# chrhansk/pygradflow

Hardware: AMD Instinct MI355X
Metric: Newton steps/sec on dense KKT n=4096 m=1024; iterate match <=1e-10 (higher is better)
Workload: dtype f64; 1 GPU; dense_qp_n4096_m1024; n=4096, m=1024, newton_type=Full, step_solver=Symmetric, instances_per_gpu=1, collective=none

## Files before the change

include/pgf_hip.h:

```cpp
#ifndef PGF_HIP_H
#define PGF_HIP_H

#include <stdint.h>

#ifdef __cplusplus
extern "C" {
#endif

#define PGF_OK 0
#define PGF_SINGULAR 1
#define PGF_INERTIA 2
#define PGF_INVALID 3
#define PGF_NOT_READY 4
#define PGF_HIP_ERROR 100

#define PGF_HOST 0
#define PGF_DEVICE 1

#define PGF_CREATE_SPARSE 1u

#define PGF_STEP_RECOMPUTE_MASK 1u
#define PGF_STEP_REFACTOR 2u
#define PGF_STEP_REFACTOR_ON_CHANGE 4u

// ... 121 lines not shown
                     double *flops_out);

int pgf_kkt_apply(pgf_handle h, const double *v, double *out);

int pgf_set_refinement(pgf_handle h, int mode, double tol, double fail_tol);
int pgf_refinement_stats(pgf_handle h, int *refined, int *lu_fallbacks, double *last_rel_residual);

int pgf_debug_fail_next_chain(pgf_handle h);
int pgf_debug_chain_enable(int on);
int pgf_debug_fail_next_helper(pgf_handle h);
int pgf_batch_debug_fail_next_helper(pgf_batch b);
int pgf_debug_chain_helpers(int on);
int pgf_debug_factor_kind(pgf_handle h);
int pgf_batch_debug_factor_kind(pgf_batch b);
int pgf_debug_step_stats(pgf_handle h, int *host_syncs, int *redone_steps);

#ifdef __cplusplus
}
#endif
#endif
```

pygradflow_amd/_lib.py:

```python

from __future__ import annotations

import ctypes as C
import os
import sys

import numpy as np

from .errors import LinearSolverError

_HERE = os.path.dirname(os.path.abspath(__file__))
LIB_PATH = os.path.join(_HERE, "libpgf_hip.so")

PGF_OK, PGF_SINGULAR, PGF_INERTIA, PGF_INVALID, PGF_NOT_READY, PGF_HIP_ERROR = 0, 1, 2, 3, 4, 100
PGF_HOST, PGF_DEVICE = 0, 1
STEP_RECOMPUTE_MASK, STEP_REFACTOR, STEP_REFACTOR_ON_CHANGE = 1, 2, 4
CREATE_SPARSE = 1

_dp = C.POINTER(C.c_double)
_u8p = C.POINTER(C.c_uint8)
_ip = C.POINTER(C.c_int)
_h = C.c_void_p

SIGNATURES = {
# ... 57 lines not shown
    "pgf_ls_destroy": (C.c_int, [_h]),
    "pgf_bench_update": (C.c_int, [C.c_int, C.c_int, C.c_int, C.c_int, C.c_int, _dp, _dp]),
    "pgf_profile_read_ex": (C.c_int, [_h, _dp, C.c_int]),
    "pgf_batch_ctl_init": (C.c_int, [_h, C.c_double, C.c_double, _dp, C.c_int]),
    "pgf_batch_ctl_iterate": (C.c_int, [_h, C.c_uint, C.c_double, C.c_int]),
    "pgf_batch_ctl_read": (C.c_int, [_h, _dp, C.POINTER(C.c_uint8), _dp, C.c_int]),
    "pgf_kkt_apply": (C.c_int, [_h, _dp, _dp]),
    "pgf_set_refinement": (C.c_int, [_h, C.c_int, C.c_double, C.c_double]),
    "pgf_refinement_stats": (C.c_int, [_h, _ip, _ip, _dp]),
    "pgf_debug_fail_next_chain": (C.c_int, [_h]),
    "pgf_debug_chain_enable": (C.c_int, [C.c_int]),
    "pgf_debug_fail_next_helper": (C.c_int, [_h]),
    "pgf_debug_chain_helpers": (C.c_int, [C.c_int]),
    "pgf_debug_factor_kind": (C.c_int, [_h]),
    "pgf_debug_step_stats": (C.c_int, [_h, _ip, _ip]),
    "pgf_batch_refinement_stats": (C.c_int, [_h, _ip]),
    "pgf_comm_unique_id": (C.c_int, [C.c_void_p]),
    "pgf_comm_create": (C.c_int, [C.c_int, C.c_int, C.c_void_p, C.c_int, C.POINTER(C.c_void_p)]),
    "pgf_comm_destroy": (C.c_int, [C.c_void_p]),
    "pgf_batch_allgather_norms": (C.c_int, [_h, C.c_void_p, C.c_void_p]),
    "pgf_batch_debug_fail_next_helper": (C.c_int, [_h]),
    "pgf_batch_debug_factor_kind": (C.c_int, [_h]),
}

_lib = None


def load():
    global _lib
    if _lib is not None:
# ... 65 lines not shown
```

pygradflow_amd/csrc/pgf_api.hip:

```cpp
#include <cmath>
#include <cstdio>
#include <cstring>
#include <new>
#include <utility>

#include "../../include/pgf_hip.h"
#include "pgf_internal.h"
#include "pgf_kernels.h"
#include "pgf_sparse.h"

#define PGF_GEMVT_PARTS 32

#define STAT_COPY 16
#define STAT_ALLOC 17

struct pgf_solver {
  int n = 0, m = 0, device = 0;
  hipStream_t stream = nullptr;
  std::string err = "";
  double dt = 0, lamb = 0, rho = 0, fact = 0, delta = 0;
  bool bounds_set = false, outer_set = false, derivs_set = false, mask_set = false;
  bool qp_mode = false, point_set = false, eval_fresh = false;
  int nI = 0, nA = 0, N = 0;
  double *H = nullptr, *J = nullptr;
// ... 36 lines not shown
  bool sp_guarded = false;
  double *h_bred = nullptr;
  bool sp_stat_pending = false;
  double *stat = nullptr, *h_stat = nullptr;
  unsigned *ticket = nullptr;
  int stat_bits = 0;
  bool counts_known = false, spec_pending = false;
  bool step_took_inject = false;
  int stat_host_syncs = 0, stat_redone = 0;
  uint8_t *h_mask_stage = nullptr;
  hipEvent_t mask_ev = nullptr;
  bool fused_eval_done = false;
  bool condensed = false;
  bool condensed_veto = false;
  double *cd_t = nullptr;
};

struct pgf_linsolver {
  int N = 0, device = 0;
  bool symmetric = true;
  hipStream_t stream = nullptr;
  DenseLdlt fac;
  DenseLu lu;
  double *rhs = nullptr, *sol = nullptr;
};

static const char *k_no_handle = "null handle";
static const char *k_chain_msg = "chained triangular solve failed its placement / timeout check "
                                 "and so did the per-block solve that replaced it";

// ... 115 lines not shown
  }
  h->fac.prof = &h->prof;
  *out = h;
  return PGF_OK;
}

int pgf_destroy(pgf_handle h) {
  if (!h) return PGF_OK;
  (void)hipSetDevice(h->device);
  if (h->stream) (void)hipStreamSynchronize(h->stream);
  ldlt_chain_timing_dump();
  void *ptrs[] = {h->csr_ptr, h->csr_idx, h->csr_val, h->Hown, h->Jown, h->lb,  h->ub,   h->slb,  h->sub,      h->xhat, h->yhat,
                  h->x,    h->y,    h->xn,  h->yn,   h->g,    h->c,        h->F,    h->b0full,
                  h->rhs,  h->sol,  h->dx,  h->dy,   h->q,    h->b,        h->w,    h->tmpn,
                  h->partial, h->red, h->stat, h->mask, h->mask_new, h->idxI, h->idxA, h->pos,
                  h->meas, h->rs_v, h->rs_lv, h->rs_u, h->rs_wy, h->rs_r, h->rs_d, h->cd_t};
  for (void *p : ptrs)
    if (p) (void)hipFree(p);
  if (h->h_stat) (void)hipHostFree(h->h_stat);
  if (h->h_mask_stage) (void)hipHostFree(h->h_mask_stage);
  if (h->mask_ev) (void)hipEventDestroy(h->mask_ev);
  if (h->h_bred) (void)hipHostFree(h->h_bred);
  lu_free(h->lu);
  if (h->h_meas) (void)hipHostFree(h->h_meas);
  {
    SparseDev &sp = h->sp;
    void *sps[] = {sp.pos, sp.Hptr, sp.Hrow, sp.Hcol, sp.Hslot, sp.Jptr, sp.Jcol, sp.Jslot, sp.JTptr,
                   sp.JTrow, sp.JTmap, sp.Hval, sp.Jval, sp.band, sp.brhs, sp.Hb0, sp.Jb0,
                   sp.bD, sp.bL, sp.bU, sp.bDinv, sp.bF, sp.bneg, sp.brhs0, sp.bres, sp.bsol,
                   sp.bred};
    for (void *q : sps)
// ... 14 lines not shown
  return PGF_OK;
}

static int up(pgf_handle h, void *dst, const void *src, size_t bytes) {
  if (!bytes) return PGF_OK;
  HIPCHK(h, hipMemcpyAsync(dst, src, bytes, hipMemcpyHostToDevice, h->stream));
  return PGF_OK;
}

static int down(pgf_handle h, void *dst, const void *src, size_t bytes) {
  if (!bytes) return PGF_OK;
  HIPCHK(h, hipMemcpyAsync(dst, src, bytes, hipMemcpyDeviceToHost, h->stream));
  return PGF_OK;
}

static void invalidate_factor(pgf_handle h) {
  h->fac.factored = false;
  h->condensed_veto = false;
  h->lu_active = false;
  h->factor_clean = false;
}

int pgf_set_bounds(pgf_handle h, const double *lb, const double *ub) {
  if (!h) return PGF_INVALID;
  if (h->n && (!lb || !ub)) return fail(h, PGF_INVALID, "null bounds");
  (void)hipSetDevice(h->device);
  int rc;
  if ((rc = up(h, h->lb, lb, h->n * sizeof(double)))) return rc;
  if ((rc = up(h, h->ub, ub, h->n * sizeof(double)))) return rc;
  HIPCHK(h, hipStreamSynchronize(h->stream));
// ... 45 lines not shown
  HIPCHK(h, hipStreamSynchronize(h->stream));
  *cur = *own;
  *curld = cols;
  *owned = true;
  return PGF_OK;
}

int pgf_set_derivs_dense(pgf_handle h, const double *H, int64_t ldh, const double *J, int64_t ldj,
                         int loc) {
  if (!h) return PGF_INVALID;
  (void)hipSetDevice(h->device);
  int rc;
  if ((rc = set_matrix(h, H, ldh, h->n, h->n, loc, &h->Hown, &h->H, &h->ldh, &h->ownH))) return rc;
  if ((rc = set_matrix(h, J, ldj, h->m, h->n, loc, &h->Jown, &h->J, &h->ldj, &h->ownJ))) return rc;
  h->derivs_set = true;
  h->norms_valid = false;
  invalidate_factor(h);
  return PGF_OK;
}

static int csr_matrix_to_dense(pgf_handle h, int rows, int cols, const int *ptr, const int *idx,
                               const double *val, double **own, double **cur, int64_t *curld,
                               bool *owned) {
  if (rows == 0 || cols == 0) {
    *cur = nullptr;
    *curld = cols;
    return PGF_OK;
  }
  if (!ptr) return fail(h, PGF_INVALID, "null CSR row pointer");
  const int nnz = ptr[rows];
  if (ptr[0] != 0 || nnz < 0 || (nnz && (!idx || !val)))
// ... 35 lines not shown
}

int pgf_set_derivs_csr(pgf_handle h, const int *Hptr, const int *Hidx, const double *Hval,
                       const int *Jptr, const int *Jidx, const double *Jval) {
  if (!h) return PGF_INVALID;
  if (h->sparse) return fail(h, PGF_INVALID, "banded handles take pgf_sparse_set_pattern / _values");
  (void)hipSetDevice(h->device);
  int rc;
  if ((rc = csr_matrix_to_dense(h, h->n, h->n, Hptr, Hidx, Hval, &h->Hown, &h->H, &h->ldh,
                                &h->ownH)))
    return rc;
  if ((rc = csr_matrix_to_dense(h, h->m, h->n, Jptr, Jidx, Jval, &h->Jown, &h->J, &h->ldj,
                                &h->ownJ)))
    return rc;
  h->derivs_set = true;
  h->norms_valid = false;
  invalidate_factor(h);
  return PGF_OK;
}

static void tau_factors(pgf_handle h, double tau, int *use_tau, double *f_x, double *f_x0,
                        double *f_d) {
  *use_tau = std::isnan(tau) ? 0 : 1;
  const double lamb = 1.0 / h->dt;
  *f_x = *use_tau ? lamb * (1 - tau * lamb) : 0.0;
  *f_x0 = *use_tau ? tau * lamb * lamb : 0.0;
  *f_d = *use_tau ? tau * lamb : 0.0;
}

int pgf_active_set(pgf_handle h, const double *x, const double *g, double tau, uint8_t *mask_out) {
  if (!h) return PGF_INVALID;
// ... 139 lines not shown
    f.V = nullptr;
    f.vcap = 0;
    if ((e = hipMalloc((void **)&f.V, need * sizeof(double))) != hipSuccess) return e;
    f.vcap = need;
  }
  if (f.vdcap < (size_t)mp) {
    if (f.vd) (void)hipFree(f.vd);
    f.vd = nullptr;
    f.vdcap = 0;
    if ((e = hipMalloc((void **)&f.vd, (size_t)mp * sizeof(double))) != hipSuccess) return e;
    f.vdcap = mp;
  }
  return e;
}

static hipError_t kkt_solve_async(pgf_handle h, const double *rhs, double *sol) {
  if (!h->condensed) return ldlt_solve_async(h->fac, rhs, sol);
  DenseLdlt &f = h->fac;
  launch_cond_rhs(h->stream, h->nI, h->m, f.V, f.ldv, rhs, h->delta, h->cd_t);
  hipError_t e = ldlt_solve_async(f, h->cd_t, sol);
  if (e != hipSuccess) return e;
  launch_cond_y(h->stream, h->nI, h->m, f.V, f.ldv, sol, rhs + h->nI, h->delta, h->partial,
                (size_t)PGF_GEMVT_PARTS * (h->n ? h->n : 1), sol + h->nI);
  return hipGetLastError();
}
static hipError_t kkt_backsolve_async(pgf_handle h, double *sol) {
  DenseLdlt &f = h->fac;
  if (!h->condensed) return ldlt_backsolve_async(f, f.K + (int64_t)h->N * f.ldk, sol);
  hipError_t e = ldlt_backsolve_async(f, f.K + (int64_t)h->nI * f.ldk, sol);
  if (e != hipSuccess) return e;
// ... 22 lines not shown
  if (h->sparse) {
    sp_launch_assemble(h->stream, h->sp, h->n, h->m, h->mask, h->lamb, h->delta);
    if (sp_cyclic(h->sp)) {
      sp_cyclic_solve(h->stream, h->sp, h->n + h->m, h->fac.flags, false);
    } else {
      sp_launch_factor(h->stream, h->sp, h->n + h->m, h->fac.flags);
    }
    HIPCHK(h, hipMemcpyAsync(h->fac.h_flags, h->fac.flags, 4 * sizeof(int), hipMemcpyDeviceToHost,
                             h->stream));
    h->fac.factored = false;
    return PGF_OK;
  }
  h->lu_active = false;
  h->condensed = condensed_wanted(h);
  h->fac.vdepth = 0;
  if (h->condensed) {
    DenseLdlt &f = h->fac;
    HIPCHK(h, condensed_reserve(h));
    const int nI = h->nI, mp = (h->m + 31) / 32 * 32;
    f.ldv = condensed_ldv(h->m);
    f.vdepth = mp;
    f.vneg = h->m;
    f.flags_zeroed = nI > 0;
    launch_assemble_kkt(h->stream, f.K, f.ldk, h->H, h->ldh, h->J, h->ldj, h->idxI, nI, 0, h->lamb, h->delta,
                        f.flags, 4 + LDLT_UPD_COUNTERS, with_rhs ? h->rhs : nullptr,
                        f.K + (int64_t)nI * f.ldk, nI);
    launch_cond_panel(h->stream, f.V, f.ldv, mp, f.vd, h->J, h->ldj, h->idxI, nI, h->m, h->delta,
                      with_rhs ? h->rhs + nI : nullptr);
    HIPCHK(h, ldlt_factor_async(f, nI, nI + (with_rhs ? 1 : 0)));
    f.N = nI;
    return PGF_OK;
  }
  h->fac.flags_zeroed = h->N > 0;
  launch_assemble_kkt(h->stream, h->fac.K, h->fac.ldk, h->H, h->ldh, h->J, h->ldj, h->idxI, h->nI, h->m,
                      h->lamb, h->delta, h->fac.flags, 4 + LDLT_UPD_COUNTERS, with_rhs ? h->rhs : nullptr,
                      h->fac.K + (int64_t)h->N * h->fac.ldk, h->N);
  HIPCHK(h, ldlt_factor_async(h->fac, h->N, h->N + (with_rhs ? 1 : 0)));
  return PGF_OK;
}

#define PGF_RETRY_FACTOR (-2)
static int finish_factor_state(pgf_handle h, hipError_t *e) {
  const int st = ldlt_finish(h->fac, e);
  if (st == 1 && h->condensed && !h->condensed_veto) {
    h->condensed_veto = true;
    h->fac.factored = false;
    return 2;
  }
  return st;
}
static const char *k_helper_msg =
    "the dense factorisation failed its hand-over checks with and without helper workgroups";

static int sparse_status_sync(pgf_handle h) {
  if (!h->sparse || !h->sp_stat_pending) return PGF_OK;
  HIPCHK(h, hipStreamSynchronize(h->stream));
  h->sp_stat_pending = false;
  const int nr = h->sp.nred;
  double sum = 0.0;
  for (int i = 0; i < nr; ++i) sum += h->h_bred[2 * nr + i];
  h->h_scal[0] = sqrt(sum);
  for (int k = 0; k < 4; ++k) h->fac.h_flags[k] = (int)h->h_bred[3 * nr + k];
  return PGF_OK;
// ... 221 lines not shown
}

int pgf_factor(pgf_handle h, int *n_neg) {
  if (!h) return PGF_INVALID;
  int rc;
  if ((rc = check_ready(h))) return rc;
  (void)hipSetDevice(h->device);
  if ((rc = factor_sync(h))) return rc;
  if (n_neg) *n_neg = h->fac.n_neg;
  return PGF_OK;
}

static int newton_core_async(pgf_handle h, bool *did_factor) {
  hipStream_t s = h->stream;
  h->fused_eval_done = false;
  const bool rhs_fused = !h->sparse && h->nA == 0;
  if (rhs_fused)
    launch_residual_rhs(s, h->n, h->m, h->nI, h->lamb, h->dt, h->fact, h->xhat, h->yhat, h->x, h->y, h->g,
                        h->c, h->slb, h->sub, h->mask, h->idxI, h->F, h->b0full, h->rhs);
  else
    launch_residual(s, h->n, h->m, h->lamb, h->dt, h->xhat, h->yhat, h->x, h->y, h->g, h->c, h->slb,
                    h->sub, h->mask, h->F, h->b0full);
  if (h->sparse) {
    const int Nf = h->n + h->m;
    sp_launch_rhs(s, h->sp, h->n, h->m, h->mask, h->F, h->b0full, h->fact, h->sp.Hb0, h->sp.Jb0);
    *did_factor = false;
    if (sp_cyclic(h->sp)) {
      if (!h->fac.factored) sp_launch_assemble(s, h->sp, h->n, h->m, h->mask, h->lamb, h->delta);
      hipEvent_t e0 = nullptr, e1 = nullptr;
      if (h->prof.enabled) {
// ... 572 lines not shown
  if (!h->sparse) return down(h, h->h_stat, h->stat, STAT_COPY * sizeof(double));
  if (!h->sp_stat_pending) return down(h, h->h_scal, h->scal, sizeof(double));
  return PGF_OK;
}

static int settle_spec(pgf_handle h, bool *redone) {
  *redone = false;
  if (h->sparse || !h->step_pending || !h->spec_pending) return PGF_OK;
  h->spec_pending = false;
  if (!h->h_counts[3]) return PGF_OK;
  ++h->stat_redone;
  const int *w = reinterpret_cast<const int *>(h->h_stat + 14);
  ldlt_chain_discard(h->fac, (h->stat_bits & 2) ? w[3] : 0);
  h->stat_bits = 0;
  if (h->step_took_inject) h->fac.inject_helper_failure = 1;
  h->fac.factored = false;
  h->lu_active = false;
  std::swap(h->x, h->xn);
  std::swap(h->y, h->yn);
  h->eval_fresh = false;
  h->nI = h->h_counts[0];
  h->nA = h->h_counts[1];
  h->N = h->nI + h->m;
  int rc;
  if ((rc = enqueue_qp_step(h))) return rc;
  *redone = true;
  return PGF_OK;
}

int pgf_qp_step_async(pgf_handle h, unsigned policy, double tau) {
// ... 84 lines not shown
int pgf_debug_chain_enable(int on) {
  ldlt_chain_set_enabled(on != 0);
  return PGF_OK;
}

int pgf_debug_fail_next_helper(pgf_handle h) {
  if (!h) return PGF_INVALID;
  h->fac.inject_helper_failure = 1;
  return PGF_OK;
}

int pgf_debug_step_stats(pgf_handle h, int *host_syncs, int *redone_steps) {
  if (!h) return PGF_INVALID;
  if (host_syncs) *host_syncs = h->stat_host_syncs;
  if (redone_steps) *redone_steps = h->stat_redone;
  return PGF_OK;
}

int pgf_debug_factor_kind(pgf_handle h) {
  if (!h || h->sparse) return 0;
  if (h->lu_active) return 3;
  if (!h->fac.factored) return 0;
  return h->condensed ? 2 : 1;
}

int pgf_debug_chain_helpers(int on) {
  const int was = ldlt_chain_helpers_enabled() ? 1 : 0;
  if (on == 0 || on == 1) ldlt_chain_helpers_set(on == 1);
  return was;
}
// ... 520 lines not shown
static int batch_repair_instance(pgf_batch b, int i, double *diff_out) {
  pgf_handle h = b->hs[i];
  if (h->sparse || !h->refine_mode) return PGF_SINGULAR;
  const int nI = b->h_flags[3 * i + 2];
  h->nI = nI;
  h->nA = h->n - nI;
  h->N = nI + h->m;
  h->mask_set = true;
  h->condensed = b->cond_last;
  h->lu_active = false;
  h->last_solve = 2;
  DenseLdlt &f = h->fac;
  f.N = h->condensed ? nI : h->N;
  f.vdepth = h->condensed ? b->cond_mp : 0;
  f.ldv = condensed_ldv(h->m);
  f.vneg = h->m;
  f.factored = true;
  f.n_neg = b->h_flags[3 * i + 1] + (h->condensed ? h->m : 0);
  enqueue_residual(h);
  hipError_t e = hipStreamSynchronize(h->stream);
  if (e != hipSuccess) return hip_fail(h, e, "batched repair");
  int rc = refine_if_needed(h, false, false);
  if (rc) return rc;
  enqueue_step_update(h);
  launch_copy(h->stream, h->x, h->xn, h->n);
  launch_copy(h->stream, h->y, h->yn, h->m);
  if ((e = hipMemcpyAsync(h->h_scal, h->scal, sizeof(double), hipMemcpyDeviceToHost, h->stream)) != hipSuccess ||
      (e = hipStreamSynchronize(h->stream)) != hipSuccess)
    return hip_fail(h, e, "batched repair");
  if (ldlt_chain_check(f)) return fail(h, PGF_HIP_ERROR, k_chain_msg);
  *diff_out = h->h_scal[0];
// ... 499 lines not shown
```

pygradflow_amd/csrc/pgf_factor2.hip:

```cpp
#include <hip/hip_ext.h>

#include "pgf_internal.h"
#include "pgf_ldlt_dev.h"

#include <algorithm>
#include <atomic>
#include <cstdio>
#include <cstdlib>
#include <unordered_map>
#include <vector>

#define C_LD 66
#define C_WLD 18
#define CH_ROWS 256
#define CH_WAVES 16
#define CH_LT_OFF (CH_ROWS * C_LD * 8 + 2 * 64 * C_WLD * 8 + 3 * 64 * 8 + 16)
#define CH_SMEM (CH_LT_OFF + 2 * 16 * 16 * 8)

template <int TS>
__device__ __forceinline__ void tile_msub(double4_t &acc, double (*As)[C_LD], double (*Bs)[C_LD],
                                          const double *A, int64_t lda, int i0, int ilim,
                                          const double *B, int64_t ldb, int j0, int jlim, int kd) {
  constexpr int WPR = TS / 16, NT = 64 * WPR * WPR, NQ = TS * 32 / NT;
  const int tid = threadIdx.x, lane = tid & 63, wave = tid >> 6;
// ... 1935 lines not shown
    launch_t(c1, f.W + (size_t)(buf ^ 1) * f.wstride);
  }
  if (p) (void)hipEventRecord(p->factor_spans.back().second, s);
  if (f.inject_helper_failure) {
    f.inject_helper_failure = 0;
    hipLaunchKernelGGL(k_helper_inject, dim3(1), dim3(1), 0, s, f.flags);
  }
  if (f.defer_status) {
    f.status_words |= 1;
  } else {
    e = hipMemcpyAsync(f.h_flags, f.flags, 4 * sizeof(int), hipMemcpyDeviceToHost, s);
    if (e != hipSuccess) return e;
  }
  return hipGetLastError();
}
```

pygradflow_amd/csrc/pgf_internal.h:

```cpp
#pragma once

#include <hip/hip_runtime.h>
#include <stdint.h>

#include <string>
#include <vector>

#define PGF_NB 64

struct PgfProfile {
  bool enabled = false;
  int mode = 1;
  std::vector<std::pair<hipEvent_t, hipEvent_t>> fused_spans, trsmud_spans;
  std::vector<double> fused_flops, fused_bytes;
  double acc_fused_ms = 0, acc_fused_flops = 0, acc_fused_bytes = 0, acc_trsmud_ms = 0;
  int64_t acc_fused_launches = 0;
  std::vector<hipEvent_t> pool;
  std::vector<std::pair<hipEvent_t, hipEvent_t>> update_spans;
  std::vector<double> update_flops;
  std::vector<double> update_bytes;
  std::vector<std::pair<hipEvent_t, hipEvent_t>> factor_spans;
  std::vector<std::pair<hipEvent_t, hipEvent_t>> chain_spans, trsm_spans, udiag_spans;
  double acc_update_ms = 0, acc_update_flops = 0, acc_update_bytes = 0, acc_factor_ms = 0;
  double acc_chain_ms = 0, acc_trsm_ms = 0, acc_udiag_ms = 0;
// ... 30 lines not shown
  double *vd = nullptr;
  int vdepth = 0;
  int vneg = 0;
  size_t vcap = 0, vdcap = 0;
  int inject_chain_failure = 0;
  int inject_helper_failure = 0;
  bool flags_zeroed = false;
  bool defer_status = false;
  int status_words = 0;
};

hipError_t ldlt_alloc(DenseLdlt &f, int Nmax, hipStream_t stream);
void ldlt_free(DenseLdlt &f);
void ldlt_chain_discard(DenseLdlt &f, int word);
hipError_t ldlt_factor_async(DenseLdlt &f, int N, int nrows);
int ldlt_finish(DenseLdlt &f, hipError_t *err);
hipError_t ldlt_solve_async(DenseLdlt &f, const double *rhs, double *sol);
hipError_t ldlt_backsolve_async(DenseLdlt &f, const double *w, double *sol);
int ldlt_chain_check(DenseLdlt &f);
void ldlt_chain_set_enabled(bool on);
void ldlt_chain_helpers_off();
void ldlt_inject_helper_failure(hipStream_t s, int *flags);
bool ldlt_chain_helpers_enabled();
void ldlt_chain_helpers_set(bool on);
void ldlt_chain_timing_dump();
hipEvent_t prof_event(PgfProfile *p);

struct DenseLu {
  int N = 0;
  int64_t ld = 0;
// ... 110 lines not shown
```

pygradflow_amd/csrc/pgf_kernels.h:

```cpp
#pragma once

#include <hip/hip_runtime.h>
#include <stdint.h>

void launch_scale_bounds(hipStream_t s, int n, double lamb, const double *lb, const double *ub,
                         double *slb, double *sub);
void launch_active_set(hipStream_t s, int n, int use_tau, double lamb, double f_x, double f_x0,
                       double f_d, const double *xhat, const double *x, const double *g,
                       const double *slb, const double *sub, uint8_t *mask);
void launch_compact(hipStream_t s, int n, const uint8_t *mask, int *idxI, int *idxA, int *pos,
                    int *counts, int expect);
void launch_mask_compact(hipStream_t s, int n, int use_tau, double lamb, double f_x, double f_x0,
                         double f_d, const double *xhat, const double *x, const double *g,
                         const double *slb, const double *sub, uint8_t *mask, int *idxI, int *idxA,
                         int *pos, int *counts, int expect);
void launch_residual(hipStream_t s, int n, int m, double lamb, double dt, const double *xhat,
                     const double *yhat, const double *x, const double *y, const double *g,
                     const double *c, const double *slb, const double *sub, const uint8_t *mask,
                     double *F, double *b0full);
void launch_residual_rhs(hipStream_t s, int n, int m, int nI, double lamb, double dt, double fact,
                         const double *xhat, const double *yhat, const double *x, const double *y,
                         const double *g, const double *c, const double *slb, const double *sub,
                         const uint8_t *mask, const int *idxI, double *F, double *b0full, double *rhs);
void launch_reduced_rhs(hipStream_t s, int n, int m, int nI, int nA, double fact, const double *F,
                        const int *idxI, const int *idxA, const double *H, int64_t ldh, const double *J,
                        int64_t ldj, const double *b0full, double *partial, int nparts, double *rhs);
void launch_assemble_kkt(hipStream_t s, double *K, int64_t ldk, const double *H, int64_t ldh,
                         const double *J, int64_t ldj, const int *idxI, int nI, int m,
                         double lamb, double delta, int *zero = nullptr, int nzero = 0,
                         const double *row_src = nullptr, double *row_dst = nullptr, int row_n = 0);
void launch_copy(hipStream_t s, double *dst, const double *src, int n);
void launch_copy_u8(hipStream_t s, uint8_t *dst, const uint8_t *src, int n);
void launch_mask_diff(hipStream_t s, int n, const uint8_t *a, const uint8_t *b, int *out);
int step_update_blocks(int n, int m);
void launch_step_update(hipStream_t s, int n, int m, int nI, double fact, double rho,
                        const double *x, const double *y, const double *lb, const double *ub,
                        const uint8_t *mask, const int *pos, const double *b0full,
                        const double *F, const double *sol, double *dx, double *dy, double *xn,
                        double *yn, double *red, double *diff_out, unsigned *ticket, double lamb = 0.0,
                        double *v = nullptr, double *lv = nullptr, double *zero3 = nullptr,
                        const int *flags_src = nullptr, const int *chain_src = nullptr,
                        int *status = nullptr);
void launch_gemv_rows(hipStream_t s, int rows, int cols, const double *M, int64_t ld,
                      const double *v, const double *add, double sgn, double *out);
void launch_gemvT(hipStream_t s, int rows, int cols, const double *M, int64_t ld,
// ... 37 lines not shown
```

pygradflow_amd/csrc/pgf_kernels.hip:

```cpp
#include "pgf_kernels.h"

#include <algorithm>

#include "pgf_internal.h"

#define ACTIVE_EPS 1e-8

__device__ __forceinline__ void b_scale_bounds(int n, double lamb, const double *__restrict__ lb,
                               const double *__restrict__ ub, double *__restrict__ slb,
                               double *__restrict__ sub) {
  const int i = blockIdx.x * blockDim.x + threadIdx.x;
  if (i < n) {
    slb[i] = lamb * lb[i];
    sub[i] = lamb * ub[i];
  }
}

__device__ __forceinline__ uint8_t active_flag(int i, int use_tau, double lamb, double f_x,
                                               double f_x0, double f_d,
                                               const double *__restrict__ xhat,
                                               const double *__restrict__ x,
                                               const double *__restrict__ g,
                                               const double *__restrict__ slb,
                                               const double *__restrict__ sub) {
// ... 162 lines not shown
    double corr = 0.0;
    if (nA > 0) {
      corr = lane < nparts ? partial[(int64_t)lane * n + gi] : 0.0;
      corr = wave_sum(corr);
    }
    if (lane == 0) rhs[i] = F[gi] - corr;
    return;
  }
  const int r = i - nI;
  double corr = 0.0;
  if (nA > 0) corr = row_dot(J + (int64_t)r * ldj, b0full, n, lane);
  if (lane == 0) rhs[i] = fact * F[n + r] - corr;
}

#define ASM_ROWS 8
template <int ROWS = ASM_ROWS>
__device__ __forceinline__ void b_assemble_kkt(double *__restrict__ K, int64_t ldk,
                                               const double *__restrict__ H, int64_t ldh,
                                               const double *__restrict__ J, int64_t ldj,
                                               const int *__restrict__ idxI, int nI, int m,
                                               double lamb, double delta) {
  const int N = nI + m;
  const int i0 = blockIdx.y * ROWS;
  const int j = blockIdx.x * 256 + threadIdx.x;
  if ((int)blockIdx.x * 256 >= N || (int)blockIdx.x * 256 > i0 + ROWS - 1) return;
  const int gj = (j < nI) ? idxI[j] : 0;
  static_assert(ROWS <= 64, "one lane per row of the workgroup");
  const int lane = threadIdx.x & 63;
  const int rowidx = (lane < ROWS && i0 + lane < nI) ? idxI[i0 + lane] : 0;
  constexpr int G = ROWS < 8 ? ROWS : 8;
#pragma unroll
  for (int r0 = 0; r0 < ROWS; r0 += G) {
    double v[G];
#pragma unroll
    for (int u = 0; u < G; ++u) {
      const int i = i0 + r0 + u;
      const int gi = __builtin_amdgcn_readlane(rowidx, r0 + u);
      v[u] = 0.0;
      if (i < N && j <= i && j < N) {
        if (i < nI) {
          v[u] = H[(int64_t)gi * ldh + gj];
        } else if (j < nI) {
          v[u] = J[(int64_t)(i - nI) * ldj + gj];
        }
      }
    }
#pragma unroll
    for (int u = 0; u < G; ++u) {
      const int i = i0 + r0 + u;
      if (i < N && j <= i && j < N) {
        double w = v[u];
        if (i == j) w = (i < nI) ? w + lamb : -delta;
        K[(int64_t)i * ldk + j] = w;
      }
    }
  }
}

__device__ __forceinline__ void b_copy(double *__restrict__ dst, const double *__restrict__ src,
    int n) {
  const int i = blockIdx.x * blockDim.x + threadIdx.x;
  if (i < n) dst[i] = src[i];
}

__device__ __forceinline__ void b_copy_u8(uint8_t *__restrict__ dst,
    const uint8_t *__restrict__ src, int n) {
// ... 271 lines not shown
  b_reduced_rhs(n, m, nI, nA, fact, F, idxI, J, ldj, b0full, partial, nparts, rhs);
}

__global__ __launch_bounds__(256) void k_assemble_kkt(double *__restrict__ K, int64_t ldk,
    const double *__restrict__ H, int64_t ldh, const double *__restrict__ J, int64_t ldj,
    const int *__restrict__ idxI, int nI, int m, double lamb, double delta, int *__restrict__ zero,
    int nzero, const double *__restrict__ row_src, double *__restrict__ row_dst, int row_n) {
  if (blockIdx.y == 0) {
    if (zero && blockIdx.x == 0)
      for (int t = threadIdx.x; t < nzero; t += 256) zero[t] = 0;
    const int j = blockIdx.x * 256 + threadIdx.x;
    if (row_src && j < row_n) row_dst[j] = row_src[j];
  }
  b_assemble_kkt(K, ldk, H, ldh, J, ldj, idxI, nI, m, lamb, delta);
}

__global__ void k_copy(double *__restrict__ dst, const double *__restrict__ src, int n) {
  b_copy(dst, src, n);
}

__global__ void k_copy_u8(uint8_t *__restrict__ dst, const uint8_t *__restrict__ src, int n) {
  b_copy_u8(dst, src, n);
}

__global__ void k_mask_diff(int n, const uint8_t *__restrict__ a, const uint8_t *__restrict__ b,
    int *__restrict__ out) {
  b_mask_diff(n, a, b, out);
}

__device__ __forceinline__ bool last_block_reduce(const double *red, int nb, double *out,
// ... 139 lines not shown
void launch_reduced_rhs(hipStream_t s, int n, int m, int nI, int nA, double fact, const double *F,
                        const int *idxI, const int *idxA, const double *H, int64_t ldh, const double *J,
                        int64_t ldj, const double *b0full, double *partial, int nparts, double *rhs) {
  const int N = nI + m;
  if (!N) return;
  if (nA > 0 && nI > 0)
    hipLaunchKernelGGL(k_active_rows_partial, dim3((n + 255) / 256, nparts), dim3(256), 0, s, n, nA, idxA,
                       H, ldh, b0full, nparts, partial);
  hipLaunchKernelGGL(k_reduced_rhs, dim3((N + 3) / 4), dim3(256), 0, s, n, m, nI, nA, fact, F, idxI, J,
                     ldj, b0full, partial, nparts, rhs);
}

void launch_assemble_kkt(hipStream_t s, double *K, int64_t ldk, const double *H, int64_t ldh,
                         const double *J, int64_t ldj, const int *idxI, int nI, int m,
                         double lamb, double delta, int *zero, int nzero, const double *row_src,
                         double *row_dst, int row_n) {
  const int N = nI + m;
  if (N)
    hipLaunchKernelGGL(k_assemble_kkt, dim3((N + 255) / 256, (N + ASM_ROWS - 1) / ASM_ROWS),
                       dim3(256), 0, s, K, ldk, H, ldh, J, ldj, idxI, nI, m, lamb, delta, zero, nzero,
                       row_src, row_dst, std::min(row_n, N));
}

void launch_copy(hipStream_t s, double *dst, const double *src, int n) {
  if (n) hipLaunchKernelGGL(k_copy, g1(n), dim3(256), 0, s, dst, src, n);
}

void launch_copy_u8(hipStream_t s, uint8_t *dst, const uint8_t *src, int n) {
  if (n) hipLaunchKernelGGL(k_copy_u8, g1(n), dim3(256), 0, s, dst, src, n);
}

void launch_mask_diff(hipStream_t s, int n, const uint8_t *a, const uint8_t *b, int *out) {
  if (n) hipLaunchKernelGGL(k_mask_diff, g1(n), dim3(256), 0, s, n, a, b, out);
}

int step_update_blocks(int n, int m) { return (n + m + 255) / 256; }
// ... 943 lines not shown
```

pygradflow_amd/csrc/pgf_ldlt.hip:

```cpp
#include <hip/hip_ext.h>

#include "pgf_internal.h"

#include <algorithm>
#include <cmath>
#include <cstdlib>

#include "pgf_ldlt_dev.h"

__device__ long long g_upd_clk[4];

template <int BM, int BN, int BK, int WR = 2, int WC = 2, int DB = 0, int EXP = 0>
__global__ __launch_bounds__(64 * WR * WC) void k_ldlt_update(
    double *__restrict__ K, int64_t ldk, const double *__restrict__ W, int64_t ldw, int N,
    int nrows, int row0, int col0, int colEnd, int kc0, int KB) {
  __shared__ __attribute__((aligned(16))) unsigned char smem[(DB ? 2 : 1) * (BM + BN) * (BK + 2) * 8];
  const int bx = blockIdx.x, by = blockIdx.y;
  const int i0 = row0 + by * BM;
  const int j0 = col0 + bx * BN;
  if (j0 > i0 + BM - 1) return;
  const bool stamp = (EXP & 32) && threadIdx.x == 0 && bx == 0 && by == (int)gridDim.y / 2;
  if (stamp) {
    g_upd_clk[0] = clock64();
    g_upd_clk[1] = wall_clock64();
// ... 527 lines not shown
  (void)hipEventCreate(&e);
  return e;
}

int ldlt_finish(DenseLdlt &f, hipError_t *err) {
  hipError_t e = hipStreamSynchronize(f.stream);
  if (err) *err = e;
  if (e != hipSuccess) return -1;
  ldlt_chain_timing_dump();
  if (f.h_flags[2]) {
    f.h_flags[2] = 0;
    ldlt_chain_helpers_off();
    f.factored = false;
    return 2;
  }
  f.n_neg = f.h_flags[1] + (f.vdepth > 0 ? f.vneg : 0);
  f.factored = (f.h_flags[0] == 0);
  return f.h_flags[0] ? 1 : 0;
}

static bool g_chain_off = false;
static bool use_chain() {
  static const bool on = !(getenv("PGF_TRSV_CHAIN") && atoi(getenv("PGF_TRSV_CHAIN")) == 0);
  return on && !g_chain_off;
}

void ldlt_chain_set_enabled(bool on) { g_chain_off = !on; }
bool ldlt_chain_enabled() { return use_chain(); }

int ldlt_chain_check(DenseLdlt &f) {
  if (!f.chain || !f.h_flags) return 0;
// ... 280 lines not shown
```

Measured before the change: 525.8 Newton steps/s.

## Cache full Gram matrix J^T J for condensed factorisation across Newton steps

```diff
diff --git a/include/pgf_hip.h b/include/pgf_hip.h
--- a/include/pgf_hip.h
+++ b/include/pgf_hip.h
@@ -159,6 +159,7 @@
 int pgf_debug_factor_kind(pgf_handle h);
 int pgf_batch_debug_factor_kind(pgf_batch b);
 int pgf_debug_step_stats(pgf_handle h, int *host_syncs, int *redone_steps);
+int pgf_debug_gram_stats(pgf_handle h, int *builds, int *factorisations_with_gram);
 
 #ifdef __cplusplus
 }
diff --git a/pygradflow_amd/_lib.py b/pygradflow_amd/_lib.py
--- a/pygradflow_amd/_lib.py
+++ b/pygradflow_amd/_lib.py
@@ -95,6 +95,7 @@
     "pgf_debug_chain_helpers": (C.c_int, [C.c_int]),
     "pgf_debug_factor_kind": (C.c_int, [_h]),
     "pgf_debug_step_stats": (C.c_int, [_h, _ip, _ip]),
+    "pgf_debug_gram_stats": (C.c_int, [_h, _ip, _ip]),
     "pgf_batch_refinement_stats": (C.c_int, [_h, _ip]),
     "pgf_comm_unique_id": (C.c_int, [C.c_void_p]),
     "pgf_comm_create": (C.c_int, [C.c_int, C.c_int, C.c_void_p, C.c_int, C.POINTER(C.c_void_p)]),
diff --git a/pygradflow_amd/csrc/pgf_api.hip b/pygradflow_amd/csrc/pgf_api.hip
--- a/pygradflow_amd/csrc/pgf_api.hip
+++ b/pygradflow_amd/csrc/pgf_api.hip
@@ -74,6 +74,13 @@
   bool condensed = false;
   bool condensed_veto = false;
   double *cd_t = nullptr;
+  double *G = nullptr;
+  int64_t ldg = 0;
+  int *gram_aux = nullptr;
+  bool gram_valid = false, gram_off = false;
+  int cond_since_upload = 0;
+  bool fac_counted = false, fac_used_gram = false;
+  int stat_gram_builds = 0, stat_gram_factors = 0;
 };
 
 struct pgf_linsolver {
@@ -219,7 +226,8 @@
                   h->x,    h->y,    h->xn,  h->yn,   h->g,    h->c,        h->F,    h->b0full,
                   h->rhs,  h->sol,  h->dx,  h->dy,   h->q,    h->b,        h->w,    h->tmpn,
                   h->partial, h->red, h->stat, h->mask, h->mask_new, h->idxI, h->idxA, h->pos,
-                  h->meas, h->rs_v, h->rs_lv, h->rs_u, h->rs_wy, h->rs_r, h->rs_d, h->cd_t};
+                  h->meas, h->rs_v, h->rs_lv, h->rs_u, h->rs_wy, h->rs_r, h->rs_d, h->cd_t,
+                  h->G,    h->gram_aux};
   for (void *p : ptrs)
     if (p) (void)hipFree(p);
   if (h->h_stat) (void)hipHostFree(h->h_stat);
@@ -264,6 +272,12 @@
   return PGF_OK;
 }
 
+static void invalidate_derivs(pgf_handle h) {
+  h->norms_valid = false;
+  h->gram_valid = false;
+  h->cond_since_upload = 0;
+}
+
 static void invalidate_factor(pgf_handle h) {
   h->fac.factored = false;
   h->condensed_veto = false;
@@ -339,7 +353,7 @@
   if ((rc = set_matrix(h, H, ldh, h->n, h->n, loc, &h->Hown, &h->H, &h->ldh, &h->ownH))) return rc;
   if ((rc = set_matrix(h, J, ldj, h->m, h->n, loc, &h->Jown, &h->J, &h->ldj, &h->ownJ))) return rc;
   h->derivs_set = true;
-  h->norms_valid = false;
+  invalidate_derivs(h);
   invalidate_factor(h);
   return PGF_OK;
 }
@@ -405,7 +419,7 @@
                                 &h->ownJ)))
     return rc;
   h->derivs_set = true;
-  h->norms_valid = false;
+  invalidate_derivs(h);
   invalidate_factor(h);
   return PGF_OK;
 }
@@ -575,6 +589,56 @@
   return e;
 }
 
+static int gram_mode() {
+  static const int v = []() {
+    const char *e = getenv("PGF_CONDENSED_GRAM");
+    return e ? atoi(e) : 1;
+  }();
+  return v;
+}
+static bool gram_prepare(pgf_handle h) {
+  const int mode = gram_mode();
+  if (!mode || h->gram_off) return false;
+  if (h->gram_valid) return true;
+  if (mode == 1 && h->cond_since_upload < 1) return false;
+  DenseLdlt &f = h->fac;
+  const int n = h->n, mp = (h->m + 31) / 32 * 32;
+  if (!h->G) {
+    int64_t ld = ((int64_t)n + 15) / 16 * 16;
+    if (ld % 512 == 0) ld += 16;
+    std::vector<int> ident((size_t)n + 1, 0);
+    for (int i = 0; i < n; ++i) ident[i] = i;
+    if (hipMalloc((void **)&h->G, (size_t)n * ld * sizeof(double)) != hipSuccess ||
+        hipMalloc((void **)&h->gram_aux, ((size_t)n + 1) * sizeof(int)) != hipSuccess ||
+        hipMemcpy(h->gram_aux, ident.data(), ((size_t)n + 1) * sizeof(int), hipMemcpyHostToDevice) != hipSuccess) {
+      (void)hipGetLastError();
+      if (h->G) (void)hipFree(h->G);
+      if (h->gram_aux) (void)hipFree(h->gram_aux);
+      h->G = nullptr;
+      h->gram_aux = nullptr;
+      h->gram_off = true;
+      return false;
+    }
+    h->ldg = ld;
+  }
+  launch_cond_panel(h->stream, f.V, condensed_ldv(h->m), mp, f.vd, h->J, h->ldj, h->gram_aux, n, h->m, 1.0,
+                    nullptr);
+  if (ldlt_gram_async(h->stream, h->G, h->ldg, n, f.V, condensed_ldv(h->m), f.vd, mp, h->gram_aux + n) !=
+      hipSuccess) {
+    (void)hipGetLastError();
+    h->gram_off = true;
+    return false;
+  }
+  h->gram_valid = true;
+  ++h->stat_gram_builds;
+  return true;
+}
+static void gram_uncount(pgf_handle h) {
+  if (h->fac_counted) --h->cond_since_upload;
+  if (h->fac_used_gram) --h->stat_gram_factors;
+  h->fac_counted = h->fac_used_gram = false;
+}
+
 static hipError_t kkt_solve_async(pgf_handle h, const double *rhs, double *sol) {
   if (!h->condensed) return ldlt_solve_async(h->fac, rhs, sol);
   DenseLdlt &f = h->fac;
@@ -627,14 +691,32 @@
   h->lu_active = false;
   h->condensed = condensed_wanted(h);
   h->fac.vdepth = 0;
+  h->fac.vneg = 0;
+  h->fac_counted = h->fac_used_gram = false;
   if (h->condensed) {
     DenseLdlt &f = h->fac;
     HIPCHK(h, condensed_reserve(h));
     const int nI = h->nI, mp = (h->m + 31) / 32 * 32;
     f.ldv = condensed_ldv(h->m);
+    f.vneg = h->m;
+    const bool gram = gram_prepare(h);
+    ++h->cond_since_upload;
+    h->fac_counted = true;
+    f.flags_zeroed = nI > 0;
+    if (gram) {
+      ++h->stat_gram_factors;
+      h->fac_used_gram = true;
+      launch_assemble_kkt(h->stream, f.K, f.ldk, h->H, h->ldh, h->J, h->ldj, h->idxI, nI, 0, h->lamb, h->delta,
+                          f.flags, 4 + LDLT_UPD_COUNTERS, nullptr, nullptr, 0, h->G, h->ldg);
+      launch_cond_panel(h->stream, f.V, f.ldv, mp, f.vd, h->J, h->ldj, h->idxI, nI, h->m, h->delta,
+                        with_rhs ? h->rhs + nI : nullptr);
+      if (with_rhs)
+        launch_cond_rhs(h->stream, nI, h->m, f.V, f.ldv, h->rhs, h->delta, f.K + (int64_t)nI * f.ldk);
+      HIPCHK(h, ldlt_factor_async(f, nI, nI + (with_rhs ? 1 : 0)));
+      f.N = nI;
+      return PGF_OK;
+    }
     f.vdepth = mp;
-    f.vneg = h->m;
-    f.flags_zeroed = nI > 0;
     launch_assemble_kkt(h->stream, f.K, f.ldk, h->H, h->ldh, h->J, h->ldj, h->idxI, nI, 0, h->lamb, h->delta,
                         f.flags, 4 + LDLT_UPD_COUNTERS, with_rhs ? h->rhs : nullptr,
                         f.K + (int64_t)nI * f.ldk, nI);
@@ -658,8 +740,10 @@
   if (st == 1 && h->condensed && !h->condensed_veto) {
     h->condensed_veto = true;
     h->fac.factored = false;
+    gram_uncount(h);
     return 2;
   }
+  if (st == 2) gram_uncount(h);
   return st;
 }
 static const char *k_helper_msg =
@@ -911,6 +995,7 @@
 static int newton_core_async(pgf_handle h, bool *did_factor) {
   hipStream_t s = h->stream;
   h->fused_eval_done = false;
+  h->fac_counted = h->fac_used_gram = false;
   const bool rhs_fused = !h->sparse && h->nA == 0;
   if (rhs_fused)
     launch_residual_rhs(s, h->n, h->m, h->nI, h->lamb, h->dt, h->fact, h->xhat, h->yhat, h->x, h->y, h->g,
@@ -1513,6 +1598,7 @@
   ldlt_chain_discard(h->fac, (h->stat_bits & 2) ? w[3] : 0);
   h->stat_bits = 0;
   if (h->step_took_inject) h->fac.inject_helper_failure = 1;
+  gram_uncount(h);
   h->fac.factored = false;
   h->lu_active = false;
   std::swap(h->x, h->xn);
@@ -1627,6 +1713,13 @@
   if (!h) return PGF_INVALID;
   if (host_syncs) *host_syncs = h->stat_host_syncs;
   if (redone_steps) *redone_steps = h->stat_redone;
+  return PGF_OK;
+}
+
+int pgf_debug_gram_stats(pgf_handle h, int *builds, int *factorisations_with_gram) {
+  if (!h) return PGF_INVALID;
+  if (builds) *builds = h->stat_gram_builds;
+  if (factorisations_with_gram) *factorisations_with_gram = h->stat_gram_factors;
   return PGF_OK;
 }
 
@@ -2177,7 +2270,7 @@
   f.N = h->condensed ? nI : h->N;
   f.vdepth = h->condensed ? b->cond_mp : 0;
   f.ldv = condensed_ldv(h->m);
-  f.vneg = h->m;
+  f.vneg = h->condensed ? h->m : 0;
   f.factored = true;
   f.n_neg = b->h_flags[3 * i + 1] + (h->condensed ? h->m : 0);
   enqueue_residual(h);
diff --git a/pygradflow_amd/csrc/pgf_factor2.hip b/pygradflow_amd/csrc/pgf_factor2.hip
--- a/pygradflow_amd/csrc/pgf_factor2.hip
+++ b/pygradflow_amd/csrc/pgf_factor2.hip
@@ -7,6 +7,7 @@
 #include <atomic>
 #include <cstdio>
 #include <cstdlib>
+#include <cstring>
 #include <unordered_map>
 #include <vector>
 
@@ -1973,3 +1974,35 @@
   }
   return hipGetLastError();
 }
+
+hipError_t ldlt_gram_async(hipStream_t s, double *G, int64_t ldg, int n, const double *V, int64_t ldv,
+                           const double *vd, int depth, int *ctr) {
+  if (n <= 0 || depth <= 0 || depth % 32) return hipErrorInvalidValue;
+  hipError_t e;
+  if ((e = hipMemsetAsync(G, 0, (size_t)n * ldg * sizeof(double), s)) != hipSuccess) return e;
+  if ((e = hipMemsetAsync(ctr, 0, sizeof(int), s)) != hipSuccess) return e;
+  static const int ncu = []() {
+    int dev = 0, c = 256;
+    hipDeviceProp_t pr;
+    if (hipGetDevice(&dev) == hipSuccess && hipGetDeviceProperties(&pr, dev) == hipSuccess && pr.multiProcessorCount > 0)
+      c = pr.multiProcessorCount;
+    return c;
+  }();
+  UpdJobs js;
+  memset(&js, 0, sizeof js);
+  js.njobs = 1;
+  js.col0[0] = 0;
+  js.rowstart[0] = 0;
+  js.kc0[0] = 0;
+  js.KB[0] = 0;
+  js.kc0v[0] = 0;
+  js.KBv[0] = depth;
+  js.ntc[0] = (n + 127) / 128;
+  int ntiles = 0;
+  for (int c = 0; c < js.ntc[0]; ++c) ntiles += (n - 128 * c + UPD_TM - 1) / UPD_TM;
+  js.tile_begin[0] = 0;
+  js.tile_begin[1] = ntiles;
+  const UpdVirt uv{V, ldv, vd};
+  hipLaunchKernelGGL(k_update_jobs, dim3(std::min(ntiles, ncu)), dim3(1024), 0, s, G, ldg, G, n, n, js, uv, ctr);
+  return hipGetLastError();
+}
diff --git a/pygradflow_amd/csrc/pgf_internal.h b/pygradflow_amd/csrc/pgf_internal.h
--- a/pygradflow_amd/csrc/pgf_internal.h
+++ b/pygradflow_amd/csrc/pgf_internal.h
@@ -68,6 +68,8 @@
 void ldlt_free(DenseLdlt &f);
 void ldlt_chain_discard(DenseLdlt &f, int word);
 hipError_t ldlt_factor_async(DenseLdlt &f, int N, int nrows);
+hipError_t ldlt_gram_async(hipStream_t s, double *G, int64_t ldg, int n, const double *V, int64_t ldv,
+                           const double *vd, int depth, int *ctr);
 int ldlt_finish(DenseLdlt &f, hipError_t *err);
 hipError_t ldlt_solve_async(DenseLdlt &f, const double *rhs, double *sol);
 hipError_t ldlt_backsolve_async(DenseLdlt &f, const double *w, double *sol);
diff --git a/pygradflow_amd/csrc/pgf_kernels.h b/pygradflow_amd/csrc/pgf_kernels.h
--- a/pygradflow_amd/csrc/pgf_kernels.h
+++ b/pygradflow_amd/csrc/pgf_kernels.h
@@ -28,7 +28,8 @@
 void launch_assemble_kkt(hipStream_t s, double *K, int64_t ldk, const double *H, int64_t ldh,
                          const double *J, int64_t ldj, const int *idxI, int nI, int m,
                          double lamb, double delta, int *zero = nullptr, int nzero = 0,
-                         const double *row_src = nullptr, double *row_dst = nullptr, int row_n = 0);
+                         const double *row_src = nullptr, double *row_dst = nullptr, int row_n = 0,
+                         const double *G = nullptr, int64_t ldg = 0);
 void launch_copy(hipStream_t s, double *dst, const double *src, int n);
 void launch_copy_u8(hipStream_t s, uint8_t *dst, const uint8_t *src, int n);
 void launch_mask_diff(hipStream_t s, int n, const uint8_t *a, const uint8_t *b, int *out);
diff --git a/pygradflow_amd/csrc/pgf_kernels.hip b/pygradflow_amd/csrc/pgf_kernels.hip
--- a/pygradflow_amd/csrc/pgf_kernels.hip
+++ b/pygradflow_amd/csrc/pgf_kernels.hip
@@ -200,12 +200,14 @@
 }
 
 #define ASM_ROWS 8
-template <int ROWS = ASM_ROWS>
+template <int ROWS = ASM_ROWS, bool GRAM = false>
 __device__ __forceinline__ void b_assemble_kkt(double *__restrict__ K, int64_t ldk,
                                                const double *__restrict__ H, int64_t ldh,
                                                const double *__restrict__ J, int64_t ldj,
                                                const int *__restrict__ idxI, int nI, int m,
-                                               double lamb, double delta) {
+                                               double lamb, double delta,
+                                               const double *__restrict__ G = nullptr, int64_t ldg = 0,
+                                               double ginv = 0.0) {
   const int N = nI + m;
   const int i0 = blockIdx.y * ROWS;
   const int j = blockIdx.x * 256 + threadIdx.x;
@@ -214,28 +216,31 @@
   static_assert(ROWS <= 64, "one lane per row of the workgroup");
   const int lane = threadIdx.x & 63;
   const int rowidx = (lane < ROWS && i0 + lane < nI) ? idxI[i0 + lane] : 0;
-  constexpr int G = ROWS < 8 ? ROWS : 8;
+  constexpr int GR = ROWS < 8 ? ROWS : 8;
 #pragma unroll
-  for (int r0 = 0; r0 < ROWS; r0 += G) {
-    double v[G];
+  for (int r0 = 0; r0 < ROWS; r0 += GR) {
+    double v[GR], vg[GR];
 #pragma unroll
-    for (int u = 0; u < G; ++u) {
+    for (int u = 0; u < GR; ++u) {
       const int i = i0 + r0 + u;
       const int gi = __builtin_amdgcn_readlane(rowidx, r0 + u);
       v[u] = 0.0;
+      if (GRAM) vg[u] = 0.0;
       if (i < N && j <= i && j < N) {
         if (i < nI) {
           v[u] = H[(int64_t)gi * ldh + gj];
+          if (GRAM) vg[u] = G[(int64_t)max(gi, gj) * ldg + min(gi, gj)];
         } else if (j < nI) {
           v[u] = J[(int64_t)(i - nI) * ldj + gj];
         }
       }
     }
 #pragma unroll
-    for (int u = 0; u < G; ++u) {
+    for (int u = 0; u < GR; ++u) {
       const int i = i0 + r0 + u;
       if (i < N && j <= i && j < N) {
         double w = v[u];
+        if (GRAM && i < nI) w += vg[u] * ginv;
         if (i == j) w = (i < nI) ? w + lamb : -delta;
         K[(int64_t)i * ldk + j] = w;
       }
@@ -537,6 +542,19 @@
   }
   b_assemble_kkt(K, ldk, H, ldh, J, ldj, idxI, nI, m, lamb, delta);
 }
+__global__ __launch_bounds__(256) void k_assemble_kkt_gram(double *__restrict__ K, int64_t ldk,
+    const double *__restrict__ H, int64_t ldh, const double *__restrict__ J, int64_t ldj,
+    const int *__restrict__ idxI, int nI, int m, double lamb, double delta, int *__restrict__ zero,
+    int nzero, const double *__restrict__ row_src, double *__restrict__ row_dst, int row_n,
+    const double *__restrict__ G, int64_t ldg, double ginv) {
+  if (blockIdx.y == 0) {
+    if (zero && blockIdx.x == 0)
+      for (int t = threadIdx.x; t < nzero; t += 256) zero[t] = 0;
+    const int j = blockIdx.x * 256 + threadIdx.x;
+    if (row_src && j < row_n) row_dst[j] = row_src[j];
+  }
+  b_assemble_kkt<ASM_ROWS, true>(K, ldk, H, ldh, J, ldj, idxI, nI, m, lamb, delta, G, ldg, ginv);
+}
 
 __global__ void k_copy(double *__restrict__ dst, const double *__restrict__ src, int n) {
   b_copy(dst, src, n);
@@ -706,12 +724,16 @@
 void launch_assemble_kkt(hipStream_t s, double *K, int64_t ldk, const double *H, int64_t ldh,
                          const double *J, int64_t ldj, const int *idxI, int nI, int m,
                          double lamb, double delta, int *zero, int nzero, const double *row_src,
-                         double *row_dst, int row_n) {
+                         double *row_dst, int row_n, const double *G, int64_t ldg) {
   const int N = nI + m;
-  if (N)
-    hipLaunchKernelGGL(k_assemble_kkt, dim3((N + 255) / 256, (N + ASM_ROWS - 1) / ASM_ROWS),
-                       dim3(256), 0, s, K, ldk, H, ldh, J, ldj, idxI, nI, m, lamb, delta, zero, nzero,
-                       row_src, row_dst, std::min(row_n, N));
+  if (!N) return;
+  const dim3 grid((N + 255) / 256, (N + ASM_ROWS - 1) / ASM_ROWS);
+  if (G)
+    hipLaunchKernelGGL(k_assemble_kkt_gram, grid, dim3(256), 0, s, K, ldk, H, ldh, J, ldj, idxI, nI, m, lamb,
+                       delta, zero, nzero, row_src, row_dst, std::min(row_n, N), G, ldg, 1.0 / delta);
+  else
+    hipLaunchKernelGGL(k_assemble_kkt, grid, dim3(256), 0, s, K, ldk, H, ldh, J, ldj, idxI, nI, m, lamb, delta,
+                       zero, nzero, row_src, row_dst, std::min(row_n, N));
 }
 
 void launch_copy(hipStream_t s, double *dst, const double *src, int n) {
diff --git a/pygradflow_amd/csrc/pgf_ldlt.hip b/pygradflow_amd/csrc/pgf_ldlt.hip
--- a/pygradflow_amd/csrc/pgf_ldlt.hip
+++ b/pygradflow_amd/csrc/pgf_ldlt.hip
@@ -565,7 +565,7 @@
     f.factored = false;
     return 2;
   }
-  f.n_neg = f.h_flags[1] + (f.vdepth > 0 ? f.vneg : 0);
+  f.n_neg = f.h_flags[1] + f.vneg;
   f.factored = (f.h_flags[0] == 0);
   return f.h_flags[0] ? 1 : 0;
 }
```

New measurement: 586.5 Newton steps/s (median of 6 runs). 11.6% higher.
